# segasai/rvspecfit

Hardware: AMD Instinct MI355X
Metric: spectra/sec (CCF+chi2 grid) DESI 3-arm (higher is better)
Workload: dtype f64

## Files before the change

### include/rvsgpu.h

```cpp
#ifndef RVSGPU_H
#define RVSGPU_H
#include <stdint.h>

#ifdef __cplusplus
extern "C" {
#endif

#define RVS_E_ARG (-1)
#define RVS_E_LAUNCH (-2)

#define RVS_ST_SPLINE_RANGE 0x1
#define RVS_ST_SPLINE_GRID 0x2
#define RVS_ST_NONFINITE 0x4
#define RVS_ST_CHOL_FALLBACK 0x8
#define RVS_ST_OUTSIDE_NAN 0x10
#define RVS_ST_CCF_FAILED 0x20
#define RVS_ST_ALLMASKED 0x40
#define RVS_ST_QUAD_ASSERT 0x80
#define RVS_ST_ILLCOND 0x100
#define RVS_ST_NONPOS_MEDIAN 0x200
#define RVS_ST_RBF_NOTPD 0x400

#define RVS_ABI_VERSION 18
int rvs_abi_version(void);
// ... 303 lines not shown
int rvs_grid_moments(const double *chisq, const double *vels,
                     int64_t vel_stride, const int32_t *nvel, int G, int Np,
                     int Nv, int quadratic, double *res, double *probs,
                     int32_t *status, void *stream);

int rvs_ccf_preprocess(const double *lam, const double *spec,
                       const double *espec, const uint8_t *badmask, int npix,
                       int B, int continuum, const double *Eb, const int32_t *El,
                       const double *Cinv, const int32_t *istart, int nnode,
                       const int32_t *bin_start, const int32_t *xind,
                       const double *rw, int nfft, double maxerr,
                       double *proc_spec, double *proc_ivar, double *sse,
                       double *cont, double *pfit, int32_t *status,
                       void *stream);
int rvs_ccf_preprocess_g(const double *lam, const double *spec, const double *espec,
                         const uint8_t *badmask, int npix, int B, int continuum,
                         const double *Eb, const int32_t *El, const double *Cinv,
                         const int32_t *istart, int nnode,
                         const int32_t *bin_start, const int32_t *xind,
                         const double *rw, int nfft, double maxerr,
                         double *proc_spec, double *proc_ivar, double *sse,
                         double *cont, double *pfit, int32_t *status,
                         const int32_t *grid_id, const int32_t *npix_g,
                         const int32_t *nnode_g, void *stream);

int rvs_ccf_fft_pos(int nfft, int f);
int rvs_ccf_xcorr(const double *proc_spec, const double *proc_ivar, int nfft,
                  int B, const double *tfft, const double *tfft2, int T,
                  const double *twid, int continuum, const int32_t *lag_pos,
                  const double *lag_vel, int nlag, const int32_t *ilo,
                  const double *vgrid, int nvel, double beta,
                  const uint8_t *prune, double *chisq, double *work,
                  void *stream);

#define RVS_CCF_MODEL_MAX_NTP 9216
int rvs_ccf_model_rows(const float *dats, int64_t ngrid, const int64_t *sel,
                       int exp_flag, int ntp, int M, double *rows, void *stream);
int rvs_ccf_models_build(const double *rows, const uint8_t *f32row,
                         const double *erows, int ntp, int M, int continuum,
                         const double *Eb, const int32_t *El, const double *Cinv,
                         const int32_t *istart, int nnode, const int32_t *bin_start,
                         const double *lnlam, const double *logl, const int32_t *ihi,
                         int npoints, const double *twid, double *model, double *fft,
                         double *fft2, double *cont, double *pfit, int32_t *status,
                         void *stream);

int rvs_ccf_select(const double *chisq, const double *sse, int narm_sse, int B,
                   int T, const double *vgrid, int nvel, double *res,
                   double *best_ccf, int32_t *status, void *stream);

int rvs_template_nn(const double *params, int B, int ndim, uint32_t log_mask,
                    const double *M, const double *S, int nlayer,
                    const float *const *W, const float *const *b,
                    const int32_t *dims, float *act0, float *act1,
                    double *templ, void *stream);

int rvs_template_nn_grad(const double *params, int B, int ndim, uint32_t log_mask,
                         const double *M, const double *S, int nlayer,
                         const float *const *W, const float *const *b,
                         const int32_t *dims, float *act0, float *act1,
                         double *templ , void *stream);

int rvs_nn_outside(const double *params, int B, int ndim, uint32_t log_mask,
                   const double *M, const double *S, int mapped,
                   const double *xeqs, int nfx, const double *yeqs, int nfy,
                   double *outside, void *stream);
// ... 294 lines not shown
```

### rvspecfit_amd/_lib.py

```python
import ctypes
import os

import torch

_HERE = os.path.dirname(os.path.abspath(__file__))
LIB_PATH = os.path.join(_HERE, 'librvsgpu.so')

P = ctypes.c_void_p
I = ctypes.c_int
L = ctypes.c_int64
D = ctypes.c_double
U = ctypes.c_uint32

SIGNATURES = {
    'rvs_abi_version': (I, []),
    'rvs_option_set': (I, [ctypes.c_char_p, I]),
    'rvs_option_get': (I, [ctypes.c_char_p, P]),
    'rvs_template_polylinear': (I, [P, L, I, P, P, P, I, P, P, U, I, P, I, P, P,
                                    P, P, P]),
    'rvs_template_polylinear_grad': (I, [P, L, I, P, P, P, I, P, P, U, I, P, I, P,
                                         P, P, P, P]),
    'rvs_template_tri': (I, [P, I, P, P, P, I, I, U, I, P, I, P, P, P, P, P]),
    'rvs_template_tri_buckets': (I, [P, I, P, P, P, I, I, U, I, P, P, I, P, P, P,
                                     P, P]),
# ... 76 lines not shown
    'rvs_lm_run': (I, [P, P, P, P, I, P, P]),
    'rvs_epoch_map': (I, [I, I, I, I, P, P, P, P, P, I, P, P, P, P, P, D, D, D, P, P, P,
                          P, P, P, P, P]),
    'rvs_epoch_finish': (I, [I, I, I, I, P, I, P, P, P, P, P, P, P, P, P, P, P, P, I, P,
                             P, D, P, P, P]),
    'rvs_alm_row_size': (L, [I, I]),
    'rvs_alm_begin': (P, [I, I, P, P, D, D, D, D, I]),
    'rvs_alm_pending': (L, [P, P, P, L]),
    'rvs_alm_feed': (I, [P, P, L]),
    'rvs_alm_result': (I, [P, P, P, P, P, P, P, P, P, P]),
    'rvs_alm_end': (None, [P]),
    'rvs_alm_run_bytes': (L, []),
    'rvs_alm_run': (I, [P, P, P, P]),
    'rvs_objective_max_ntp': (I, [I]),
    'rvs_objective_resol_ok': (I, [I, I, I, I]),
    'rvs_objective_work_size': (L, [I, I]),
    'rvs_objective_fused': (I, [P, I, I, P, P, P, I, P, D, I, P, P, P, P]),
    'rvs_objective_from_template': (I, [P, I, I, P, P, P, P, I, P, D, I, P, P, P,
                                        P]),
    'rvs_objective_fused_n': (I, [P, I, I, P, P, P, I, P, P, D, I, P, P, P, P]),
    'rvs_objective_from_template_n': (I, [P, I, I, P, P, P, P, I, P, P, D, I, P,
                                          P, P, P]),
    'rvs_grid_moments': (I, [P, P, L, P, I, I, I, I, P, P, P, P]),
    'rvs_basis_build': (I, [P, P, I, I, I, I, P, P, P, P, P]),
    'rvs_ccf_tables_build': (I, [P, P, I, I, P, I, I, P, P, P, I, P, P, P, P, P, P,
                                 P]),
    'rvs_ccf_preprocess': (I, [P, P, P, P, I, I, I, P, P, P, P, I, P, P, P, I, D,
                               P, P, P, P, P, P, P]),
    'rvs_ccf_preprocess_g': (I, [P, P, P, P, I, I, I, P, P, P, P, I, P, P, P, I,
                                 D, P, P, P, P, P, P, P, P, P, P]),
    'rvs_ccf_fft_pos': (I, [I, I]),
    'rvs_ccf_xcorr': (I, [P, P, I, I, P, P, I, P, I, P, P, I, P, P, I, D, P, P,
                          P, P]),
    'rvs_ccf_select': (I, [P, P, I, I, I, P, I, P, P, P, P]),
    'rvs_ccf_model_rows': (I, [P, L, P, I, I, I, P, P]),
    'rvs_ccf_models_build': (I, [P, P, P, I, I, I, P, P, P, P, I, P, P, P, P, I, P,
                                 P, P, P, P, P, P, P]),
    'rvs_template_nn': (I, [P, I, I, U, P, P, I, P, P, P, P, P, P, P]),
    'rvs_template_nn_grad': (I, [P, I, I, U, P, P, I, P, P, P, P, P, P, P]),
    'rvs_template_nn_arms': (I, [P, I, I, I, P, P]),
    'rvs_template_nn_arms_n': (I, [P, I, P, I, I, P, P]),
    'rvs_nn_outside': (I, [P, I, I, U, P, P, I, P, I, P, I, P, P]),
    'rvs_rebin_weights': (I, [P, I, P, P, P, P, I, I, P, P]),
    'rvs_rebin_apply': (I, [P, I, L, I, I, P, P, I, P, P, P, I, I, P, P]),
    'rvs_template_normalize': (I, [P, I, I, P, I, D, D, I, I, P, P, P, P]),
    'rvs_rbf_work_size': (L, [I, I]),
    'rvs_rbf_factor': (I, [P, I, I, D, P, P, P, P]),
    'rvs_rbf_solve': (I, [P, I, L, I, I, P, P, P]),
    'rvs_rbf_eval': (I, [P, I, P, I, I, D, P, I, I, P, L, P]),
    'rvs_nn_train_work_size': (L, [I, I, I, P]),
    'rvs_nn_train_grad': (I, [P, P, I, P, I, I, P, P, P, P, P, D, P, P, P, P, P, P]),
    'rvs_nn_adam_step': (I, [I, P, P, P, P, P, P, P, P, P, D, I, P]),
    'rvs_nn_train_epoch': (I, [P, P, I, P, I, I, I, P, P, P, P, P, P, P, P, P, D, D, I,
                               P, P, P, P]),
}

_lib = None
ABI_VERSION = 18


class RvsGpuError(RuntimeError):
    pass


def lib():
    global _lib
# ... 207 lines not shown
```

### rvspecfit_amd/csrc/ccf_fft.hip

```cpp
#include "common.h"

#define XC_NT 512
#define XC_NTW(n2) ((n2) >> 3)

struct XcLds {
  int t1;
  int c0;
  int t1c;
  int ca;
  int lt;
  size_t bytes;
};
#define XW_NT1C 73
#define XW_NLT 256
#define XC_LDS_MAX (159 * 1024)
__host__ __device__ constexpr XcLds xc_lds_pair(int n2, int nlag) {
  const int t1 = n2, c0 = t1 + XC_NTW(n2);
  return {t1, c0, 0, 0, 0,
          sizeof(double2) * (size_t)c0 + sizeof(double) * 2 * (size_t)nlag};
}
__host__ __device__ constexpr XcLds xc_lds_ws(int n2, int nlag, bool ratio) {
  const int t1 = 2 * n2, c0 = t1 + XC_NTW(n2), t1c = c0 + ((nlag + 1) >> 1),
            ca = t1c + XW_NT1C, lt = ca + (ratio ? (nlag + 1) >> 1 : 0);
  return {t1, c0, t1c, ca, lt,
          sizeof(double2) * (size_t)lt + sizeof(int32_t) * (size_t)XW_NLT};
}
__host__ __device__ constexpr XcLds xc_lds_ws2(int n2, int nlag) {
  const int t1 = 4 * n2, c0 = t1 + XC_NTW(n2);
  return {t1, c0, 0, 0, 0,
          sizeof(double2) * (size_t)c0 + sizeof(double) * 2 * (size_t)nlag};
}
__host__ __device__ constexpr bool xc_lds_fits(const XcLds &L, int n2, int nimg,
                                               int nrow, int nlag, bool ws, bool ratio) {
  const size_t D2 = sizeof(double2), D = sizeof(double);
  size_t end = D2 * (size_t)nimg * n2;
  if (D2 * L.t1 < end) return false;
  end = D2 * (L.t1 + XC_NTW(n2));
  if (D2 * L.c0 < end) return false;
  end = D2 * L.c0 + D * (size_t)nrow * nlag;
  if (ws) {
    if (D2 * L.t1c < end) return false;
    end = D2 * (L.t1c + 72);
    if (D2 * L.ca < end) return false;
    end = D2 * L.ca + (ratio ? D * (size_t)nlag : 0);
    if (D2 * L.lt < end) return false;
    end = D2 * L.lt + sizeof(int32_t) * (size_t)XW_NLT;
  }
  return end <= L.bytes && L.bytes <= XC_LDS_MAX;
}
constexpr bool xc_lds_check() {
  for (int nlag = 2; nlag <= 512; nlag++)
    for (int n2 = 2048; n2 <= 4096; n2 *= 2) {
      for (int ratio = 0; ratio < 2; ratio++)
        if (!xc_lds_fits(xc_lds_ws(n2, nlag, ratio), n2, 2, 1, nlag, true, ratio))
          return false;
      if (n2 == 2048 && !xc_lds_fits(xc_lds_ws2(n2, nlag), n2, 4, 2, nlag, false, false))
        return false;
      if (!xc_lds_fits(xc_lds_pair(n2, nlag), n2, 1, 2, nlag, false, false))
        return false;
    }
  return true;
}
static_assert(xc_lds_check(), "an LDS array of a cross-correlation kernel overlaps "
                              "its neighbour or ends beyond the launch's request");

__device__ __forceinline__ double2 cmul(double2 a, double2 b) {
  return make_double2(a.x * b.x - a.y * b.y, a.x * b.y + a.y * b.x);
}
__device__ __forceinline__ double2 cadd(double2 a, double2 b) {
  return make_double2(a.x + b.x, a.y + b.y);
}
__device__ __forceinline__ double2 csub(double2 a, double2 b) {
  return make_double2(a.x - b.x, a.y - b.y);
}
template <int SIGN>
__device__ __forceinline__ double2 cmuli(double2 a) {
  return (SIGN > 0) ? make_double2(-a.y, a.x) : make_double2(a.y, -a.x);
}

__host__ __device__ inline int xc_plan(int log2n, int *rad) {
  int n = 0, l = log2n;
  while (l >= 3) {
    rad[n++] = 8;
    l -= 3;
  }
  if (l == 2) rad[n++] = 4;
  if (l == 1) rad[n++] = 2;
  return n;
// ... 519 lines not shown
    if (pre) {
      if (tid < nlag) dst[tid] = fr[pre_pos] * inv_n;
    } else {
      for (int l = tid; l < nlag; l += XB_NT) dst[l] = fr[lag_pos[l]] * inv_n;
    }
    __syncthreads();
  }
  if (!continuum) {
    for (int l = tid; l < nlag; l += XB_NT) c0[l] = -c0[l] * c0[l] / c1[l];
    __syncthreads();
  }
  if (pre) {
    if (tid < nvel) {
      const double sl = (c0[pre_lo + 1] - c0[pre_lo]) / (pre_x1 - pre_x0);
      const double val = sl * (pre_xg - pre_x0) + c0[pre_lo];
      out[tid] = (beta != 0.0) ? beta * pre_old + val : val;
    }
    XC_T(2);
    return;
  }
  for (int v = tid; v < nvel; v += XB_NT) {
    const int lo = ilo[v];
    const double x0 = lag_vel[lo], x1 = lag_vel[lo + 1];
    const double sl = (c0[lo + 1] - c0[lo]) / (x1 - x0);
    const double val = sl * (vgrid[v] - x0) + c0[lo];
    out[v] = (beta != 0.0) ? beta * out[v] + val : val;
  }
}


#define XW_NT 1024
#define XW_HALF 512

template <int SIGN, int LOG2N>
__device__ __forceinline__ void xw_pass(double2 *a, const double2 *T1, int p, int t,
                                        const double2 *Tc = nullptr) {
  const int lgM = LOG2N - 3 * p, lgMp = lgM - 3, Mp = 1 << lgMp;
  const int tws = LOG2N + 1 - lgM;
  const int blk = t >> lgMp, r = t & (Mp - 1);
  const int base = (blk << lgM) + r;
  double2 v[8];
#pragma unroll
  for (int j = 0; j < 8; j++) v[j] = a[base + Mp * j];
  dft8<SIGN>(v);
  if (Mp > 1) {
    double2 w1 = Tc ? Tc[r] : T1[r << (tws - 1)];
    if (SIGN < 0) w1.y = -w1.y;
    v[1] = cmul(v[1], w1);
    const double2 w2 = cmul(w1, w1);
    v[2] = cmul(v[2], w2);
    double2 wc = cmul(w2, w1);
    v[3] = cmul(v[3], wc);
    const double2 w4 = cmul(w2, w2);
    v[4] = cmul(v[4], w4);
    v[7] = cmul(v[7], cmul(w4, wc));
    wc = cmul(w4, w1);
    v[5] = cmul(v[5], wc);
    v[6] = cmul(v[6], cmul(w4, w2));
  }
#pragma unroll
  for (int q = 0; q < 8; q++) a[base + Mp * q] = v[q];
}

template <int LOG2N, bool RATIO>
__global__ void __launch_bounds__(XW_NT)
    ccf_xcorr_ws_kernel(const double2 *__restrict__ work,
                        const double2 *__restrict__ tfft,
                        const double2 *__restrict__ tfft2, int T,
                        const double2 *__restrict__ tw,
                        const int32_t *__restrict__ lag_pos,
                        const double *__restrict__ lag_vel, int nlag,
                        const int32_t *__restrict__ ilo,
                        const double *__restrict__ vgrid, int nvel, double beta,
                        const uint8_t *__restrict__ prune,
                        double *__restrict__ chisq) {
  extern __shared__ double2 fa[];
  constexpr int log2n = LOG2N, n2 = 1 << LOG2N, nfft = 2 * n2, npair = n2 / 2;
  constexpr int NPP = npair / XW_HALF;
  constexpr bool P12 = (LOG2N == 12);
  static_assert(LOG2N == 12 || LOG2N == 11, "plans 8,8,8,8 and 8,8,8,4 only");
  auto img = [&](int i) -> double2 * { return fa + (i & 1) * n2; };
  const XcLds lds = xc_lds_ws(n2, nlag, RATIO);
  const double2 *T1 = fa + lds.t1;
  double *c0 = reinterpret_cast<double *>(fa + lds.c0);
  double2 *T1c = fa + lds.t1c;
  double *cA = reinterpret_cast<double *>(fa + lds.ca);
  int32_t *lt = reinterpret_cast<int32_t *>(fa + lds.lt);
  const int TI = RATIO ? 2 * T : T;
  const int b = blockIdx.x, tid = threadIdx.x;
  const bool producer = tid >= XW_HALF;
  const int pt = tid & (XW_HALF - 1);
  const double inv_n = 1.0 / nfft;
  if (P12 && tid < 72)
    T1c[tid] = tid < 64 ? tw[2 * (tid << 3)] : tw[2 * ((tid - 64) << (log2n - 6))];
  xc_fill_twiddles<XW_NT>(fa + n2, n2, tw);
  XcMasks pmask = {0u, 0u, 0u};
  bool bad = !P12;
  if (P12 && !producer) {
    pmask = xc_load_masks<XW_HALF>(prune, n2);
    const int pos8 = pt & 7;
    const unsigned m = pmask.g;
    bad = m != 0 && !((pos8 == 0 && m == 0x01u) || (pos8 == 7 && m == 0x80u));
  }
  if (P12 && tid < XW_NLT) lt[tid] = -1;
  const bool fold = !__syncthreads_or(bad);
  if (P12) {
    if (fold && tid < nlag) {
      const int p = lag_pos[tid], e = (p >> 1) & 63;
      if (e == 0 || e == 63) lt[(((p >> 7) & 63) << 2) + (e ? 2 : 0) + (p & 1)] = tid;
    }
    __syncthreads();
  }
  const double2 *Sc = work + ((int64_t)b * 2) * (n2 + 1);
  const double2 *Vc = Sc + (n2 + 1);
  typedef int v4i_t __attribute__((ext_vector_type(4)));
  auto ld = [](const __amdgpu_buffer_rsrc_t &r, int off) {
    const v4i_t v = __builtin_amdgcn_raw_buffer_load_b128(r, off, 0, 0);
    return make_double2(__hiloint2double(v.y, v.x), __hiloint2double(v.w, v.z));
  };
  const int nbytes = (n2 + 1) * 16;
  if (producer) {
    double2 Sk[NPP], Vk[NPP], Sm[NPP], Vm[NPP];
#pragma unroll
    for (int u = 0; u < NPP; u++) {
      const int k = 1 + pt + u * XW_HALF, m = n2 - k;
      Sk[u] = Sc[k], Vk[u] = Vc[k], Sm[u] = Sc[m], Vm[u] = Vc[m];
    }
// ... 27 lines not shown
      const int k = 1 + ptv + u * XW_HALF, m = n2 - k;
      double2 Xk, Xm;
      if (RATIO) {
        const bool second = (tcur & 1) != 0;
        Xk = cmul(o[0], second ? Vk[u] : Sk[u]);
        Xm = cmul(o[2], second ? Vm[u] : Sm[u]);
      } else {
        const double2 p1 = cmul(o[0], Sk[u]), p2 = cmul(o[1], Vk[u]);
        Xk = make_double2(p2.x - 2 * p1.x, p2.y - 2 * p1.y);
        const double2 q1 = cmul(o[2], Sm[u]), q2 = cmul(o[3], Vm[u]);
        Xm = make_double2(q2.x - 2 * q1.x, q2.y - 2 * q1.y);
      }
      const double2 e = make_double2(Xk.x + Xm.x, Xk.y - Xm.y);
      const double2 d = make_double2(Xk.x - Xm.x, Xk.y + Xm.y);
      const double2 q = cmul(o[4], d);
      dst[k] = make_double2(e.x - q.y, e.y + q.x);
      if (m != k) dst[m] = make_double2(e.x + q.y, -e.y + q.x);
      if (u == NPP - 1 && ptv == 0) {
        double xk, xm;
        if (RATIO) {
          const bool second = (tcur & 1) != 0;
          xk = cmul(second ? dc[1] : dc[0], second ? Vc[0] : Sc[0]).x;
          xm = cmul(second ? dc[3] : dc[2], second ? Vc[n2] : Sc[n2]).x;
        } else {
          const double2 a1 = cmul(dc[0], Sc[0]), a2 = cmul(dc[1], Vc[0]);
          const double2 b1 = cmul(dc[2], Sc[n2]), b2 = cmul(dc[3], Vc[n2]);
          xk = a2.x - 2 * a1.x, xm = b2.x - 2 * b1.x;
        }
        dst[0] = make_double2(xk + xm, xk - xm);
      }
    };
    const bool two = P12 && fold;
    const int nbar = two ? 2 : 5;
    issue(0, 0, op[0]);
    if (NPP == 2) issue(0, 1, op[1]);
    for (int it = -1; it < TI; it++) {
      const int tn = it + 1;
      if (tn < TI) {
        double2 *dst = img(tn);
        {
          const int tt = RATIO ? (tn >> 1) : tn;
          const double2 *Fp = tfft + (int64_t)tt * (n2 + 1);
          const double2 *F2p = tfft2 + (int64_t)tt * (n2 + 1);
          dc[0] = Fp[0], dc[1] = F2p[0], dc[2] = Fp[n2], dc[3] = F2p[n2];
        }
        if (NPP == 2) {
#pragma unroll
          for (int u = 0; u < 2; u++) {
            form(dst, u, op[u], tn);
            if (tn + 1 < TI) issue(tn + 1, u, op[u]);
            __syncthreads();
          }
        } else {
#pragma unroll
          for (int u = 0; u < NPP; u++) {
            if (u + 1 < NPP)
              issue(tn, u + 1, op[(u + 1) & 1]);
            else if (tn + 1 < TI)
              issue(tn + 1, 0, op[(u + 1) & 1]);
            form(dst, u, op[u & 1], tn);
            if (!two || (u & 1)) __syncthreads();
          }
        }
        for (int q = two ? NPP / 2 : NPP; q < nbar; q++) __syncthreads();
      } else {
        for (int q = 0; q < nbar; q++) __syncthreads();
      }
    }
    return;
  }
  const int tvx = min(pt, nvel - 1);
  const int pre_pos = lag_pos[min(pt, nlag - 1)];
  const int pre_lo = ilo[tvx];
  const double pre_xg = vgrid[tvx];
  const double pre_x0 = lag_vel[pre_lo], pre_x1 = lag_vel[pre_lo + 1];
  typedef int v4i32_t __attribute__((ext_vector_type(4)));
  v4i32_t lag = {-1, -1, -1, -1};
  if (P12) lag = reinterpret_cast<const v4i32_t *>(lt)[pt >> 3];
  for (int it = -1; it < TI; it++) {
    if (it < 0) {
      const int nbar = (P12 && fold) ? 2 : 5;
      for (int q = 0; q < nbar; q++) __syncthreads();
      continue;
    }
    double2 *a = img(it);
    double *out = chisq + ((int64_t)b * T + (RATIO ? (it >> 1) : it)) * nvel;
    double pre_old = 0;
    if (beta != 0.0) pre_old = out[tvx];
    if (pt < (n2 >> 3)) xw_pass<1, LOG2N>(a, T1, 0, pt);
    __syncthreads();
    if (pt < (n2 >> 3)) xw_pass<1, LOG2N>(a, T1, 1, pt, P12 ? T1c : nullptr);
    if (P12 && fold) {
      __builtin_amdgcn_fence(__ATOMIC_RELEASE, "wavefront");
      __builtin_amdgcn_wave_barrier();
      __builtin_amdgcn_fence(__ATOMIC_ACQUIRE, "wavefront");
      const int s = pt & 7;
      const int B = pt >> 3;
      const unsigned m0 = pmask.b0 & 1u, m63 = pmask.b7 >> 7;
      if (m0 | m63) {
        double2 v[8];
#pragma unroll
        for (int j = 0; j < 8; j++) v[j] = a[B * 64 + s + 8 * j];
        dft8<1>(v);
        double2 w = T1c[64 + s];
        w.y = -w.y;
        double2 x63 = cmul(v[7], w), x0 = v[0];
        auto sum8 = [](double x) {
          x += dpp_get<0xb1, 0xf, 0xf>(x);
          x += dpp_get<0x4e, 0xf, 0xf>(x);
          x += dpp_get<0x141, 0xf, 0xf>(x);
          return x;
        };
        auto put = [&](int l, double x) {
          if (l < 0) return;
          const double c = x * inv_n;
          if (!RATIO)
            c0[l] = c;
          else if (it & 1)
            c0[l] = -cA[l] * cA[l] / c;
          else
            cA[l] = c;
        };
        if (m0) {
          x0.x = sum8(x0.x);
// ... 200 lines not shown
    xw_pass<1, LOG2N>(a, T1, 0, bt);
    __syncthreads();
    xw_pass<1, LOG2N>(a, T1, 1, bt);
    __syncthreads();
    xw_pass<1, LOG2N>(a, T1, 2, bt);
    __syncthreads();
#pragma unroll
    for (int h = 0; h < 2; h++) {
      const int base = (bt + 256 * h) << 2;
      double2 v0 = a[base], v1 = a[base + 1], v2 = a[base + 2], v3 = a[base + 3];
      dft4<1>(v0, v1, v2, v3);
      a[base] = v0, a[base + 1] = v1, a[base + 2] = v2, a[base + 3] = v3;
    }
    __syncthreads();
    if (pt < nlag) {
      c0[pt] = reinterpret_cast<const double *>(img(it, 0))[pre_pos[0]] * inv_n;
      c0[nlag + pt] = reinterpret_cast<const double *>(img(it, 1))[pre_pos[0]] * inv_n;
    }
    __syncthreads();
    if (pt < nvel) {
      const double dx = pre_x1 - pre_x0, xg = pre_xg - pre_x0;
      const double sl0 = (c0[pre_lo + 1] - c0[pre_lo]) / dx;
      const double val0 = sl0 * xg + c0[pre_lo];
      out0[pt] = (beta != 0.0) ? beta * old0 + val0 : val0;
      if (two) {
        const double sl1 = (c0[nlag + pre_lo + 1] - c0[nlag + pre_lo]) / dx;
        const double val1 = sl1 * xg + c0[nlag + pre_lo];
        out1[pt] = (beta != 0.0) ? beta * old1 + val1 : val1;
      }
    }
  }
}

extern "C" int rvs_ccf_xcorr(const double *proc_spec, const double *proc_ivar,
                             int nfft, int B, const double *tfft,
                             const double *tfft2, int T, const double *twid_,
                             int continuum, const int32_t *lag_pos,
                             const double *lag_vel, int nlag, const int32_t *ilo,
                             const double *vgrid, int nvel, double beta,
                             const uint8_t *prune, double *chisq, double *work,
                             void *stream) {
  int log2n = 0;
  while ((2 << log2n) < nfft) log2n++;
  if ((2 << log2n) != nfft || nfft < 64 || nfft > 16384) return RVS_E_ARG;
  if (B < 1 || T < 1 || T > 65535 || nlag < 2 || nvel < 1) return RVS_E_ARG;
  const int n2 = nfft >> 1;
  const size_t shm1 = xc_lds_pair(n2, 0).bytes;
  const size_t shm2 = xc_lds_pair(n2, nlag).bytes;
  if (shm2 > XC_LDS_MAX) return RVS_E_ARG;
  hipStream_t st = rvs_stream(stream);
  const double2 *tw = reinterpret_cast<const double2 *>(twid_);
  static bool attr_set = false;
  if (!attr_set) {
    (void)hipFuncSetAttribute((const void *)ccf_rfft_kernel<false>,
                              hipFuncAttributeMaxDynamicSharedMemorySize,
                              XC_LDS_MAX);
    (void)hipFuncSetAttribute((const void *)ccf_xcorr_kernel,
                              hipFuncAttributeMaxDynamicSharedMemorySize,
                              XC_LDS_MAX);
    (void)hipGetLastError();
    attr_set = true;
  }
  hipLaunchKernelGGL(ccf_rfft_kernel<false>, dim3(B, 2), dim3(XC_NT), shm1, st,
                     proc_spec, proc_ivar, nfft, log2n, tw,
                     reinterpret_cast<double2 *>(work), (double2 *)nullptr);
  RVS_LAUNCH_CHECK();
  const int G = xc_group(T, nfft);
  {
    const bool ws_on = rvs_opt(RVS_OPT_XC_WS) != 0;
    const bool p12 = (nfft == 8192 && prune), p11 = (nfft == 4096);
    if (ws_on && (p12 || p11) && nlag <= XW_HALF && nvel <= XW_HALF && T >= 2) {
      static bool ws_attr = false;
      if (!ws_attr) {
        (void)hipFuncSetAttribute((const void *)ccf_xcorr_ws_kernel<12, false>,
                                  hipFuncAttributeMaxDynamicSharedMemorySize,
                                  XC_LDS_MAX);
        (void)hipFuncSetAttribute((const void *)ccf_xcorr_ws_kernel<12, true>,
                                  hipFuncAttributeMaxDynamicSharedMemorySize,
                                  XC_LDS_MAX);
        (void)hipFuncSetAttribute((const void *)ccf_xcorr_ws_kernel<11, true>,
                                  hipFuncAttributeMaxDynamicSharedMemorySize,
                                  XC_LDS_MAX);
        (void)hipFuncSetAttribute((const void *)ccf_xcorr_ws2_kernel,
                                  hipFuncAttributeMaxDynamicSharedMemorySize,
                                  XC_LDS_MAX);
        (void)hipGetLastError();
        ws_attr = true;
      }
      const size_t shmw = xc_lds_ws(n2, nlag, !continuum).bytes;
#define RVS_XW_ARGS                                                                 \
  reinterpret_cast<const double2 *>(work), reinterpret_cast<const double2 *>(tfft),  \
      reinterpret_cast<const double2 *>(tfft2), T, tw, lag_pos, lag_vel, nlag, ilo,  \
      vgrid, nvel, beta, prune, chisq
      if (!continuum) {
        if (p12)
          hipLaunchKernelGGL((ccf_xcorr_ws_kernel<12, true>), dim3(B), dim3(XW_NT), shmw,
                             st, RVS_XW_ARGS);
        else
          hipLaunchKernelGGL((ccf_xcorr_ws_kernel<11, true>), dim3(B), dim3(XW_NT), shmw,
                             st, RVS_XW_ARGS);
        RVS_LAUNCH_CHECK();
        return 0;
      }
      if (p12)
        hipLaunchKernelGGL((ccf_xcorr_ws_kernel<12, false>), dim3(B), dim3(XW_NT), shmw, st,
                           reinterpret_cast<const double2 *>(work),
                           reinterpret_cast<const double2 *>(tfft),
                           reinterpret_cast<const double2 *>(tfft2), T, tw, lag_pos,
                           lag_vel, nlag, ilo, vgrid, nvel, beta, prune, chisq);
      else
        hipLaunchKernelGGL(ccf_xcorr_ws2_kernel, dim3(B), dim3(XW_NT),
                           xc_lds_ws2(n2, nlag).bytes, st,
                           reinterpret_cast<const double2 *>(work),
                           reinterpret_cast<const double2 *>(tfft),
                           reinterpret_cast<const double2 *>(tfft2), T, tw, lag_pos,
                           lag_vel, nlag, ilo, vgrid, nvel, beta, chisq);
      RVS_LAUNCH_CHECK();
      return 0;
    }
  }
  const int bmax = G ? (int)(0x7fffffffll / xc_nblocks(T, 1, G)) : 65535;
  for (int b0 = 0; b0 < B; b0 += bmax) {
    const int nb = (B - b0 < bmax) ? (B - b0) : bmax;
    const dim3 grid = G ? dim3((unsigned)xc_nblocks(T, nb, G)) : dim3(T, nb);
    hipLaunchKernelGGL(
        ccf_xcorr_kernel, grid, dim3(XB_NT), shm2, st,
        reinterpret_cast<const double2 *>(work) + (int64_t)b0 * 2 * (n2 + 1),
        nfft, log2n, reinterpret_cast<const double2 *>(tfft),
        reinterpret_cast<const double2 *>(tfft2), T, tw, continuum, lag_pos,
        lag_vel, nlag, ilo, vgrid, nvel, beta, prune,
        chisq + (int64_t)b0 * T * nvel, nb, G);
    RVS_LAUNCH_CHECK();
  }
  return 0;
}
```

### rvspecfit_amd/csrc/options.cpp

```cpp
#include <atomic>
#include <cstdlib>
#include <cstring>
#include <mutex>

#include "options.h"

namespace {
struct OptDef {
  const char *name;
  const char *env;
  int dflt;
};
const OptDef kDefs[RVS_OPT_COUNT] = {
    {"xc_ws", "RVS_XC_WS", 1},
    {"obj_inblk_max", "RVS_OBJ_INBLK_MAX", 768},
    {"obj_sort", "RVS_OBJ_SORT", 1},
    {"nn_pipe", "RVS_NN_PIPE", 1},
    {"nm_split_min", "RVS_NM_SPLIT_MIN", 1024},
    {"nm_spec_max", "RVS_NM_SPEC_MAX", 21},
    {"nm_tail_window", "RVS_NM_TAIL_WINDOW", 16},
    {"cg_tab", "RVS_CG_TAB", 1},
};
std::atomic<int> g_val[RVS_OPT_COUNT];
std::once_flag g_once;

void init_table() {
  for (int i = 0; i < RVS_OPT_COUNT; i++) {
    int v = kDefs[i].dflt;
    if (const char *ev = std::getenv(kDefs[i].env))
      v = std::atoi(ev);
    g_val[i].store(v, std::memory_order_relaxed);
  }
}
int find(const char *name) {
  if (!name) return -1;
  for (int i = 0; i < RVS_OPT_COUNT; i++)
    if (!std::strcmp(name, kDefs[i].name)) return i;
  return -1;
}
}

int rvs_opt(int id) {
  std::call_once(g_once, init_table);
  return g_val[id].load(std::memory_order_relaxed);
}

extern "C" int rvs_option_set(const char *name, int value) {
  const int i = find(name);
  if (i < 0) return RVS_E_ARG;
  std::call_once(g_once, init_table);
  g_val[i].store(value, std::memory_order_relaxed);
  return 0;
}

// ... 7 lines not shown
```

### rvspecfit_amd/csrc/options.h

```cpp
#pragma once
#include "../../include/rvsgpu.h"

enum {
  RVS_OPT_XC_WS,
  RVS_OPT_OBJ_INBLK_MAX,
  RVS_OPT_OBJ_SORT,
  RVS_OPT_NN_PIPE,
  RVS_OPT_NM_SPLIT_MIN,
  RVS_OPT_NM_SPEC_MAX,
  RVS_OPT_NM_TAIL_WINDOW,
  RVS_OPT_CG_TAB,
  RVS_OPT_COUNT
};
int rvs_opt(int id);
```

### rvspecfit_amd/engine.py

```python
import ctypes
import threading

import numpy as np
import torch

from . import _lib
from . import ccf_tables

SPEED_OF_LIGHT = 299792.458

KTIMERS = None


class _ktime:

    def __init__(self, name, units=1):
        self.name, self.units = name, units

    def __enter__(self):
        if KTIMERS is not None:
            self.e0 = torch.cuda.Event(enable_timing=True)
            self.e0.record()

    def __exit__(self, *a):
# ... 1243 lines not shown
        _lib.ptr(status), arm.grid_args()[0], _lib.ptr(T['npix_g']),
        _lib.ptr(T['nnode_g']), _lib.stream())
    _lib.check(rc, 'rvs_ccf_preprocess')
    out = dict(proc_spec=ps, proc_ivar=pi, sse=sse, status=status)
    if details:
        out.update(cont=cont, pfit=pfit)
    return out


def ccf_fit(batch, libs, config, keep_all=False, max_chunk=None):
    L = _lib.lib()
    dev = batch.device
    S = batch.S
    ref = libs[batch.names[0]].ccf_set(config)
    Tn = ref['T']
    for n in batch.names[1:]:
        cc = libs[n].ccf_set(config)
        if cc['T'] != Tn:
            raise RuntimeError('CCF template counts are inconsistent across setups')
        if (not np.array_equal(ref['params'], cc['params'])
                or not np.array_equal(ref['vsinis'], cc['vsinis'],
                                      equal_nan=True)):
            raise RuntimeError('The parameters of the CCF templates do not match')
    tabs = [a.ccf_tables(libs[a.name], config) for a in batch.arms]
    nvel = len(tabs[0]['vgrid_host'])
    pre = [ccf_preprocess(a, libs[a.name], config) for a in batch.arms]
    sse = torch.stack([p['sse'] for p in pre]).contiguous()
    status = torch.zeros(S, dtype=torch.int32, device=dev)
    for p in pre:
        status |= p['status']
    if max_chunk is None:
        max_chunk = max(1, min(S, int(2e9 // (Tn * nvel * 8))))
        nchunk = -(-S // max_chunk)
        max_chunk = -(-S // nchunk)
    res = torch.empty((S, 4), dtype=torch.float64, device=dev)
    best_ccf = torch.empty((S, nvel), dtype=torch.float64, device=dev)
    allchi = None
    for a, b in _chunks(S, max_chunk):
        n = b - a
        acc = torch.empty((n, Tn, nvel), dtype=torch.float64, device=dev)
        for ia, arm in enumerate(batch.arms):
            cc = libs[arm.name].ccf_set(config)
            T = tabs[ia]
            nfft = cc['npoints']
            work = torch.empty((n, 2, nfft // 2 + 1, 2), dtype=torch.float64,
                               device=dev)
            with _ktime('ccf_xcorr', n):
              rc = L.rvs_ccf_xcorr(
                _lib.ptr(pre[ia]['proc_spec'][a:b]),
                _lib.ptr(pre[ia]['proc_ivar'][a:b]), nfft, n,
                _lib.ptr(cc['fft']), _lib.ptr(cc['fft2']), Tn,
                _lib.ptr(T['twid']), int(cc['continuum']),
                _lib.ptr(T['lag_pos']), _lib.ptr(T['lag_vel']), T['nlag'],
                _lib.ptr(T['ilo']), _lib.ptr(T['vgrid']), nvel,
                0.0 if ia == 0 else 1.0, _lib.ptr(T['prune']), _lib.ptr(acc),
                _lib.ptr(work), _lib.stream())
            _lib.check(rc, 'rvs_ccf_xcorr')
        sse_c = sse[:, a:b].contiguous()
        rc = L.rvs_ccf_select(_lib.ptr(acc), _lib.ptr(sse_c), len(batch.arms),
                              n, Tn, _lib.ptr(tabs[0]['vgrid']), nvel,
                              _lib.ptr(res[a:b]), _lib.ptr(best_ccf[a:b]),
                              _lib.ptr(status[a:b]), _lib.stream())
        _lib.check(rc, 'rvs_ccf_select')
        if keep_all:
            allchi = acc + sse_c.sum(dim=0)[:, None, None]
    out = dict(best_id=res[:, 0].long(), best_vel=res[:, 1].contiguous(),
               best_pix=res[:, 2].long(), best_ccf=best_ccf, status=status,
# ... 8 lines not shown
```

Measured before the change: 84490.

## Split tail batch blocks across templates and precompute twiddle powers in LDS

```diff
diff --git a/include/rvsgpu.h b/include/rvsgpu.h
--- a/include/rvsgpu.h
+++ b/include/rvsgpu.h
@@ -359,6 +359,8 @@
                   const double *vgrid, int nvel, double beta,
                   const uint8_t *prune, double *chisq, double *work,
                   void *stream);
+int rvs_ccf_xcorr_plan(int nfft, int B, int T, int nlag, int continuum, int ncu,
+                       int32_t *out);
 
 #define RVS_CCF_MODEL_MAX_NTP 9216
 int rvs_ccf_model_rows(const float *dats, int64_t ngrid, const int64_t *sel,
diff --git a/rvspecfit_amd/_lib.py b/rvspecfit_amd/_lib.py
--- a/rvspecfit_amd/_lib.py
+++ b/rvspecfit_amd/_lib.py
@@ -132,6 +132,7 @@
     'rvs_ccf_fft_pos': (I, [I, I]),
     'rvs_ccf_xcorr': (I, [P, P, I, I, P, P, I, P, I, P, P, I, P, P, I, D, P, P,
                           P, P]),
+    'rvs_ccf_xcorr_plan': (I, [I, I, I, I, I, I, P]),
     'rvs_ccf_select': (I, [P, P, I, I, I, P, I, P, P, P, P]),
     'rvs_ccf_model_rows': (I, [P, L, P, I, I, I, P, P]),
     'rvs_ccf_models_build': (I, [P, P, P, I, I, I, P, P, P, P, I, P, P, P, P, I, P,
diff --git a/rvspecfit_amd/csrc/ccf_fft.hip b/rvspecfit_amd/csrc/ccf_fft.hip
--- a/rvspecfit_amd/csrc/ccf_fft.hip
+++ b/rvspecfit_amd/csrc/ccf_fft.hip
@@ -5,6 +5,7 @@
 
 struct XcLds {
   int t1;
+  int p1;
   int c0;
   int t1c;
   int ca;
@@ -16,18 +17,21 @@
 #define XC_LDS_MAX (159 * 1024)
 __host__ __device__ constexpr XcLds xc_lds_pair(int n2, int nlag) {
   const int t1 = n2, c0 = t1 + XC_NTW(n2);
-  return {t1, c0, 0, 0, 0,
+  return {t1, 0, c0, 0, 0, 0,
           sizeof(double2) * (size_t)c0 + sizeof(double) * 2 * (size_t)nlag};
 }
-__host__ __device__ constexpr XcLds xc_lds_ws(int n2, int nlag, bool ratio) {
+#define XW_NP1 384
+__host__ __device__ constexpr XcLds xc_lds_ws(int n2, int nlag, bool ratio,
+                                              bool p1 = false) {
   const int t1 = 2 * n2, c0 = t1 + XC_NTW(n2), t1c = c0 + ((nlag + 1) >> 1),
-            ca = t1c + XW_NT1C, lt = ca + (ratio ? (nlag + 1) >> 1 : 0);
-  return {t1, c0, t1c, ca, lt,
-          sizeof(double2) * (size_t)lt + sizeof(int32_t) * (size_t)XW_NLT};
+            ca = t1c + XW_NT1C, lt = ca + (ratio ? (nlag + 1) >> 1 : 0),
+            pp = lt + (int)(sizeof(int32_t) * XW_NLT / sizeof(double2));
+  return {t1, p1 ? pp : 0, c0, t1c, ca, lt,
+          sizeof(double2) * (size_t)(pp + (p1 ? XW_NP1 : 0))};
 }
 __host__ __device__ constexpr XcLds xc_lds_ws2(int n2, int nlag) {
   const int t1 = 4 * n2, c0 = t1 + XC_NTW(n2);
-  return {t1, c0, 0, 0, 0,
+  return {t1, 0, c0, 0, 0, 0,
           sizeof(double2) * (size_t)c0 + sizeof(double) * 2 * (size_t)nlag};
 }
 __host__ __device__ constexpr bool xc_lds_fits(const XcLds &L, int n2, int nimg,
@@ -45,6 +49,10 @@
     end = D2 * L.ca + (ratio ? D * (size_t)nlag : 0);
     if (D2 * L.lt < end) return false;
     end = D2 * L.lt + sizeof(int32_t) * (size_t)XW_NLT;
+    if (L.p1) {
+      if (D2 * L.p1 < end) return false;
+      end = D2 * (L.p1 + XW_NP1);
+    }
   }
   return end <= L.bytes && L.bytes <= XC_LDS_MAX;
 }
@@ -52,8 +60,10 @@
   for (int nlag = 2; nlag <= 512; nlag++)
     for (int n2 = 2048; n2 <= 4096; n2 *= 2) {
       for (int ratio = 0; ratio < 2; ratio++)
-        if (!xc_lds_fits(xc_lds_ws(n2, nlag, ratio), n2, 2, 1, nlag, true, ratio))
-          return false;
+        for (int p1 = 0; p1 < (n2 == 4096 ? 2 : 1); p1++) {
+          const XcLds L = xc_lds_ws(n2, nlag, ratio, p1);
+          if (!xc_lds_fits(L, n2, 2, 1, nlag, true, ratio)) return false;
+        }
       if (n2 == 2048 && !xc_lds_fits(xc_lds_ws2(n2, nlag), n2, 4, 2, nlag, false, false))
         return false;
       if (!xc_lds_fits(xc_lds_pair(n2, nlag), n2, 1, 2, nlag, false, false))
@@ -639,9 +649,30 @@
 #define XW_NT 1024
 #define XW_HALF 512
 
+struct XwPowers {
+  double2 w2, w3, w4, w5, w6, w7;
+};
+__device__ __forceinline__ XwPowers xw_powers(double2 w1) {
+  XwPowers w;
+  w.w2 = cmul(w1, w1);
+  w.w3 = cmul(w.w2, w1);
+  w.w4 = cmul(w.w2, w.w2);
+  w.w7 = cmul(w.w4, w.w3);
+  w.w5 = cmul(w.w4, w1);
+  w.w6 = cmul(w.w4, w.w2);
+  return w;
+}
+template <bool W1>
+__device__ __forceinline__ double2 cmul_as_chain(double2 v, double2 w) {
+#pragma clang fp contract(off)
+  const double re = v.y * w.y, im = W1 ? v.x * w.y : v.y * w.x;
+  return make_double2(__builtin_fma(v.x, w.x, -re),
+                      W1 ? __builtin_fma(v.y, w.x, im) : __builtin_fma(v.x, w.y, im));
+}
 template <int SIGN, int LOG2N>
 __device__ __forceinline__ void xw_pass(double2 *a, const double2 *T1, int p, int t,
-                                        const double2 *Tc = nullptr) {
+                                        const double2 *Tc = nullptr,
+                                        const double2 *Pw = nullptr) {
   const int lgM = LOG2N - 3 * p, lgMp = lgM - 3, Mp = 1 << lgMp;
   const int tws = LOG2N + 1 - lgM;
   const int blk = t >> lgMp, r = t & (Mp - 1);
@@ -650,7 +681,11 @@
 #pragma unroll
   for (int j = 0; j < 8; j++) v[j] = a[base + Mp * j];
   dft8<SIGN>(v);
-  if (Mp > 1) {
+  if (Mp > 1 && Pw) {
+    v[1] = cmul_as_chain<true>(v[1], Tc[r]);
+#pragma unroll
+    for (int q = 2; q < 8; q++) v[q] = cmul_as_chain<false>(v[q], Pw[(q - 2) * Mp + r]);
+  } else if (Mp > 1) {
     double2 w1 = Tc ? Tc[r] : T1[r << (tws - 1)];
     if (SIGN < 0) w1.y = -w1.y;
     v[1] = cmul(v[1], w1);
@@ -669,7 +704,7 @@
   for (int q = 0; q < 8; q++) a[base + Mp * q] = v[q];
 }
 
-template <int LOG2N, bool RATIO>
+template <int LOG2N, bool RATIO, bool P1 = false>
 __global__ void __launch_bounds__(XW_NT)
     ccf_xcorr_ws_kernel(const double2 *__restrict__ work,
                         const double2 *__restrict__ tfft,
@@ -680,26 +715,41 @@
                         const int32_t *__restrict__ ilo,
                         const double *__restrict__ vgrid, int nvel, double beta,
                         const uint8_t *__restrict__ prune,
-                        double *__restrict__ chisq) {
+                        double *__restrict__ chisq, int nfull, int parts) {
   extern __shared__ double2 fa[];
   constexpr int log2n = LOG2N, n2 = 1 << LOG2N, nfft = 2 * n2, npair = n2 / 2;
   constexpr int NPP = npair / XW_HALF;
   constexpr bool P12 = (LOG2N == 12);
   static_assert(LOG2N == 12 || LOG2N == 11, "plans 8,8,8,8 and 8,8,8,4 only");
+  static_assert(P12 || !P1, "the LDS table belongs to the plan 8,8,8,8");
   auto img = [&](int i) -> double2 * { return fa + (i & 1) * n2; };
-  const XcLds lds = xc_lds_ws(n2, nlag, RATIO);
+  const XcLds lds = xc_lds_ws(n2, nlag, RATIO, P1);
   const double2 *T1 = fa + lds.t1;
   double *c0 = reinterpret_cast<double *>(fa + lds.c0);
   double2 *T1c = fa + lds.t1c;
   double *cA = reinterpret_cast<double *>(fa + lds.ca);
   int32_t *lt = reinterpret_cast<int32_t *>(fa + lds.lt);
-  const int TI = RATIO ? 2 * T : T;
-  const int b = blockIdx.x, tid = threadIdx.x;
+  double2 *Pw = P1 ? fa + lds.p1 : nullptr;
+  const int tid = threadIdx.x;
+  int b = blockIdx.x, i0 = 0, i1 = T;
+  if (b >= nfull) {
+    const int j = b - nfull, part = j % parts;
+    b = nfull + j / parts;
+    i0 = (int)((int64_t)part * T / parts), i1 = (int)((int64_t)(part + 1) * T / parts);
+  }
+  if (RATIO) i0 *= 2, i1 *= 2;
   const bool producer = tid >= XW_HALF;
   const int pt = tid & (XW_HALF - 1);
   const double inv_n = 1.0 / nfft;
-  if (P12 && tid < 72)
-    T1c[tid] = tid < 64 ? tw[2 * (tid << 3)] : tw[2 * ((tid - 64) << (log2n - 6))];
+  if (P12 && tid < 72) {
+    const double2 w1 = tid < 64 ? tw[2 * (tid << 3)] : tw[2 * ((tid - 64) << (log2n - 6))];
+    T1c[tid] = w1;
+    if (P1 && tid < 64) {
+      const XwPowers w = xw_powers(w1);
+      Pw[tid] = w.w2, Pw[64 + tid] = w.w3, Pw[128 + tid] = w.w4;
+      Pw[192 + tid] = w.w5, Pw[256 + tid] = w.w6, Pw[320 + tid] = w.w7;
+    }
+  }
   xc_fill_twiddles<XW_NT>(fa + n2, n2, tw);
   XcMasks pmask = {0u, 0u, 0u};
   bool bad = !P12;
@@ -793,11 +843,11 @@
     };
     const bool two = P12 && fold;
     const int nbar = two ? 2 : 5;
-    issue(0, 0, op[0]);
-    if (NPP == 2) issue(0, 1, op[1]);
-    for (int it = -1; it < TI; it++) {
+    issue(i0, 0, op[0]);
+    if (NPP == 2) issue(i0, 1, op[1]);
+    for (int it = i0 - 1; it < i1; it++) {
       const int tn = it + 1;
-      if (tn < TI) {
+      if (tn < i1) {
         double2 *dst = img(tn);
         {
           const int tt = RATIO ? (tn >> 1) : tn;
@@ -809,7 +859,7 @@
 #pragma unroll
           for (int u = 0; u < 2; u++) {
             form(dst, u, op[u], tn);
-            if (tn + 1 < TI) issue(tn + 1, u, op[u]);
+            if (tn + 1 < i1) issue(tn + 1, u, op[u]);
             __syncthreads();
           }
         } else {
@@ -817,7 +867,7 @@
           for (int u = 0; u < NPP; u++) {
             if (u + 1 < NPP)
               issue(tn, u + 1, op[(u + 1) & 1]);
-            else if (tn + 1 < TI)
+            else if (tn + 1 < i1)
               issue(tn + 1, 0, op[(u + 1) & 1]);
             form(dst, u, op[u & 1], tn);
             if (!two || (u & 1)) __syncthreads();
@@ -838,8 +888,8 @@
   typedef int v4i32_t __attribute__((ext_vector_type(4)));
   v4i32_t lag = {-1, -1, -1, -1};
   if (P12) lag = reinterpret_cast<const v4i32_t *>(lt)[pt >> 3];
-  for (int it = -1; it < TI; it++) {
-    if (it < 0) {
+  for (int it = i0 - 1; it < i1; it++) {
+    if (it < i0) {
       const int nbar = (P12 && fold) ? 2 : 5;
       for (int q = 0; q < nbar; q++) __syncthreads();
       continue;
@@ -850,7 +900,7 @@
     if (beta != 0.0) pre_old = out[tvx];
     if (pt < (n2 >> 3)) xw_pass<1, LOG2N>(a, T1, 0, pt);
     __syncthreads();
-    if (pt < (n2 >> 3)) xw_pass<1, LOG2N>(a, T1, 1, pt, P12 ? T1c : nullptr);
+    if (pt < (n2 >> 3)) xw_pass<1, LOG2N>(a, T1, 1, pt, P12 ? T1c : nullptr, Pw);
     if (P12 && fold) {
       __builtin_amdgcn_fence(__ATOMIC_RELEASE, "wavefront");
       __builtin_amdgcn_wave_barrier();
@@ -1117,6 +1167,63 @@
   }
 }
 
+enum { XC_FORM_PAIR, XC_FORM_WS12, XC_FORM_WS12R, XC_FORM_WS2, XC_FORM_WS11R };
+enum { XC_PLAN_FORM, XC_PLAN_ZERO, XC_PLAN_P1, XC_PLAN_LDS, XC_PLAN_FULL, XC_PLAN_REM,
+       XC_PLAN_PARTS, XC_PLAN_BLOCKS };
+static int xc_launch_plan(int nfft, int B, int T, int nlag, int nvel, int continuum,
+                          bool pruned, int ncu, int32_t out[8]) {
+  int log2n = 0;
+  while ((2 << log2n) < nfft) log2n++;
+  if ((2 << log2n) != nfft || nfft < 64 || nfft > 16384) return RVS_E_ARG;
+  if (B < 1 || T < 1 || T > 65535 || nlag < 2 || nvel < 1 || !out) return RVS_E_ARG;
+  const int n2 = nfft >> 1;
+  if (xc_lds_pair(n2, nlag).bytes > XC_LDS_MAX) return RVS_E_ARG;
+  const bool p12 = (nfft == 8192 && pruned), p11 = (nfft == 4096);
+  const bool ws = rvs_opt(RVS_OPT_XC_WS) != 0 && (p12 || p11) && nlag <= XW_HALF &&
+                  nvel <= XW_HALF && T >= 2;
+  const int64_t nblk = ws ? B : (int64_t)B * T;
+  out[XC_PLAN_FORM] = !ws ? XC_FORM_PAIR
+                      : p12 ? (continuum ? XC_FORM_WS12 : XC_FORM_WS12R)
+                            : (continuum ? XC_FORM_WS2 : XC_FORM_WS11R);
+  out[XC_PLAN_ZERO] = out[XC_PLAN_P1] = out[XC_PLAN_REM] = 0;
+  out[XC_PLAN_FULL] = ws ? B : 0;
+  out[XC_PLAN_PARTS] = 1;
+  out[XC_PLAN_BLOCKS] = (int32_t)(nblk < 0x7fffffff ? nblk : 0x7fffffff);
+  if (!ws) {
+    out[XC_PLAN_LDS] = (int32_t)xc_lds_pair(n2, nlag).bytes;
+  } else if (!p12) {
+    out[XC_PLAN_LDS] = (int32_t)(continuum ? xc_lds_ws2(n2, nlag).bytes
+                                           : xc_lds_ws(n2, nlag, true).bytes);
+  } else {
+    const XcLds L = xc_lds_ws(n2, nlag, !continuum, rvs_opt(RVS_OPT_XC_P1_LDS) != 0);
+    out[XC_PLAN_P1] = L.p1 != 0;
+    out[XC_PLAN_LDS] = (int32_t)L.bytes;
+    const int rem = ncu > 0 ? B % ncu : 0;
+    const int parts = rem ? (T < ncu / rem ? T : ncu / rem) : 1;
+    if (parts >= 2) {
+      out[XC_PLAN_FULL] = B - rem;
+      out[XC_PLAN_REM] = rem;
+      out[XC_PLAN_PARTS] = parts;
+      out[XC_PLAN_BLOCKS] = B - rem + rem * parts;
+    }
+  }
+  return 0;
+}
+
+extern "C" int rvs_ccf_xcorr_plan(int nfft, int B, int T, int nlag, int continuum,
+                                  int ncu, int32_t *out) {
+  return xc_launch_plan(nfft, B, T, nlag, 1, continuum, true, ncu, out);
+}
+
+typedef void (*XwKernel)(const double2 *, const double2 *, const double2 *, int,
+                         const double2 *, const int32_t *, const double *, int,
+                         const int32_t *, const double *, int, double, const uint8_t *,
+                         double *, int, int);
+static const XwKernel kXwKernels[5] = {
+    ccf_xcorr_ws_kernel<12, false, false>, ccf_xcorr_ws_kernel<12, false, true>,
+    ccf_xcorr_ws_kernel<12, true, false>, ccf_xcorr_ws_kernel<12, true, true>,
+    ccf_xcorr_ws_kernel<11, true>};
+
 extern "C" int rvs_ccf_xcorr(const double *proc_spec, const double *proc_ivar,
                              int nfft, int B, const double *tfft,
                              const double *tfft2, int T, const double *twid_,
@@ -1125,14 +1232,25 @@
                              const double *vgrid, int nvel, double beta,
                              const uint8_t *prune, double *chisq, double *work,
                              void *stream) {
+  int ncu = rvs_opt(RVS_OPT_XC_SPLIT_CUS);
+  int32_t plan[8];
+  int rc = xc_launch_plan(nfft, B, T, nlag, nvel, continuum, prune != nullptr, ncu, plan);
+  if (rc) return rc;
+  if (ncu == 0 &&
+      (plan[XC_PLAN_FORM] == XC_FORM_WS12 || plan[XC_PLAN_FORM] == XC_FORM_WS12R)) {
+    int dev = 0;
+    if (hipGetDevice(&dev) == hipSuccess &&
+        hipDeviceGetAttribute(&ncu, hipDeviceAttributeMultiprocessorCount, dev) ==
+            hipSuccess)
+      rc = xc_launch_plan(nfft, B, T, nlag, nvel, continuum, true, ncu, plan);
+    (void)hipGetLastError();
+  }
+  if (rc) return rc;
   int log2n = 0;
   while ((2 << log2n) < nfft) log2n++;
-  if ((2 << log2n) != nfft || nfft < 64 || nfft > 16384) return RVS_E_ARG;
-  if (B < 1 || T < 1 || T > 65535 || nlag < 2 || nvel < 1) return RVS_E_ARG;
   const int n2 = nfft >> 1;
   const size_t shm1 = xc_lds_pair(n2, 0).bytes;
   const size_t shm2 = xc_lds_pair(n2, nlag).bytes;
-  if (shm2 > XC_LDS_MAX) return RVS_E_ARG;
   hipStream_t st = rvs_stream(stream);
   const double2 *tw = reinterpret_cast<const double2 *>(twid_);
   static bool attr_set = false;
@@ -1151,58 +1269,40 @@
                      reinterpret_cast<double2 *>(work), (double2 *)nullptr);
   RVS_LAUNCH_CHECK();
   const int G = xc_group(T, nfft);
-  {
-    const bool ws_on = rvs_opt(RVS_OPT_XC_WS) != 0;
-    const bool p12 = (nfft == 8192 && prune), p11 = (nfft == 4096);
-    if (ws_on && (p12 || p11) && nlag <= XW_HALF && nvel <= XW_HALF && T >= 2) {
-      static bool ws_attr = false;
-      if (!ws_attr) {
-        (void)hipFuncSetAttribute((const void *)ccf_xcorr_ws_kernel<12, false>,
-                                  hipFuncAttributeMaxDynamicSharedMemorySize,
-                                  XC_LDS_MAX);
-        (void)hipFuncSetAttribute((const void *)ccf_xcorr_ws_kernel<12, true>,
-                                  hipFuncAttributeMaxDynamicSharedMemorySize,
-                                  XC_LDS_MAX);
-        (void)hipFuncSetAttribute((const void *)ccf_xcorr_ws_kernel<11, true>,
-                                  hipFuncAttributeMaxDynamicSharedMemorySize,
-                                  XC_LDS_MAX);
-        (void)hipFuncSetAttribute((const void *)ccf_xcorr_ws2_kernel,
-                                  hipFuncAttributeMaxDynamicSharedMemorySize,
-                                  XC_LDS_MAX);
-        (void)hipGetLastError();
-        ws_attr = true;
-      }
-      const size_t shmw = xc_lds_ws(n2, nlag, !continuum).bytes;
-#define RVS_XW_ARGS                                                                 \
-  reinterpret_cast<const double2 *>(work), reinterpret_cast<const double2 *>(tfft),  \
-      reinterpret_cast<const double2 *>(tfft2), T, tw, lag_pos, lag_vel, nlag, ilo,  \
-      vgrid, nvel, beta, prune, chisq
-      if (!continuum) {
-        if (p12)
-          hipLaunchKernelGGL((ccf_xcorr_ws_kernel<12, true>), dim3(B), dim3(XW_NT), shmw,
-                             st, RVS_XW_ARGS);
-        else
-          hipLaunchKernelGGL((ccf_xcorr_ws_kernel<11, true>), dim3(B), dim3(XW_NT), shmw,
-                             st, RVS_XW_ARGS);
-        RVS_LAUNCH_CHECK();
-        return 0;
-      }
-      if (p12)
-        hipLaunchKernelGGL((ccf_xcorr_ws_kernel<12, false>), dim3(B), dim3(XW_NT), shmw, st,
-                           reinterpret_cast<const double2 *>(work),
-                           reinterpret_cast<const double2 *>(tfft),
-                           reinterpret_cast<const double2 *>(tfft2), T, tw, lag_pos,
-                           lag_vel, nlag, ilo, vgrid, nvel, beta, prune, chisq);
-      else
-        hipLaunchKernelGGL(ccf_xcorr_ws2_kernel, dim3(B), dim3(XW_NT),
-                           xc_lds_ws2(n2, nlag).bytes, st,
-                           reinterpret_cast<const double2 *>(work),
-                           reinterpret_cast<const double2 *>(tfft),
-                           reinterpret_cast<const double2 *>(tfft2), T, tw, lag_pos,
-                           lag_vel, nlag, ilo, vgrid, nvel, beta, chisq);
-      RVS_LAUNCH_CHECK();
-      return 0;
-    }
+  const int form = plan[XC_PLAN_FORM];
+  if (form != XC_FORM_PAIR) {
+    static bool ws_attr = false;
+    if (!ws_attr) {
+      for (const XwKernel k : kXwKernels)
+        (void)hipFuncSetAttribute((const void *)k,
+                                  hipFuncAttributeMaxDynamicSharedMemorySize, XC_LDS_MAX);
+      (void)hipFuncSetAttribute((const void *)ccf_xcorr_ws2_kernel,
+                                hipFuncAttributeMaxDynamicSharedMemorySize, XC_LDS_MAX);
+      (void)hipGetLastError();
+      ws_attr = true;
+    }
+    const dim3 grid(plan[XC_PLAN_BLOCKS]);
+    const size_t shmw = plan[XC_PLAN_LDS];
+    if (form == XC_FORM_WS2) {
+      hipLaunchKernelGGL(ccf_xcorr_ws2_kernel, grid, dim3(XW_NT), shmw, st,
+                         reinterpret_cast<const double2 *>(work),
+                         reinterpret_cast<const double2 *>(tfft),
+                         reinterpret_cast<const double2 *>(tfft2), T, tw, lag_pos,
+                         lag_vel, nlag, ilo, vgrid, nvel, beta, chisq);
+    } else {
+      const XwKernel k =
+          form == XC_FORM_WS11R
+              ? kXwKernels[4]
+              : kXwKernels[2 * (form == XC_FORM_WS12R) + plan[XC_PLAN_P1]];
+      hipLaunchKernelGGL(k, grid, dim3(XW_NT), shmw, st,
+                         reinterpret_cast<const double2 *>(work),
+                         reinterpret_cast<const double2 *>(tfft),
+                         reinterpret_cast<const double2 *>(tfft2), T, tw, lag_pos,
+                         lag_vel, nlag, ilo, vgrid, nvel, beta, prune, chisq,
+                         plan[XC_PLAN_FULL], plan[XC_PLAN_PARTS]);
+    }
+    RVS_LAUNCH_CHECK();
+    return 0;
   }
   const int bmax = G ? (int)(0x7fffffffll / xc_nblocks(T, 1, G)) : 65535;
   for (int b0 = 0; b0 < B; b0 += bmax) {
diff --git a/rvspecfit_amd/csrc/options.cpp b/rvspecfit_amd/csrc/options.cpp
--- a/rvspecfit_amd/csrc/options.cpp
+++ b/rvspecfit_amd/csrc/options.cpp
@@ -20,6 +20,8 @@
     {"nm_spec_max", "RVS_NM_SPEC_MAX", 21},
     {"nm_tail_window", "RVS_NM_TAIL_WINDOW", 16},
     {"cg_tab", "RVS_CG_TAB", 1},
+    {"xc_p1_lds", "RVS_XC_P1_LDS", 1},
+    {"xc_split_cus", "RVS_XC_SPLIT_CUS", 0},
 };
 std::atomic<int> g_val[RVS_OPT_COUNT];
 std::once_flag g_once;
diff --git a/rvspecfit_amd/csrc/options.h b/rvspecfit_amd/csrc/options.h
--- a/rvspecfit_amd/csrc/options.h
+++ b/rvspecfit_amd/csrc/options.h
@@ -10,6 +10,8 @@
   RVS_OPT_NM_SPEC_MAX,
   RVS_OPT_NM_TAIL_WINDOW,
   RVS_OPT_CG_TAB,
+  RVS_OPT_XC_P1_LDS,
+  RVS_OPT_XC_SPLIT_CUS,
   RVS_OPT_COUNT
 };
 int rvs_opt(int id);
diff --git a/rvspecfit_amd/engine.py b/rvspecfit_amd/engine.py
--- a/rvspecfit_amd/engine.py
+++ b/rvspecfit_amd/engine.py
@@ -1299,7 +1299,12 @@
     if max_chunk is None:
         max_chunk = max(1, min(S, int(2e9 // (Tn * nvel * 8))))
         nchunk = -(-S // max_chunk)
+        bound = max_chunk
         max_chunk = -(-S // nchunk)
+        ncu = torch.cuda.get_device_properties(dev).multi_processor_count
+        whole = -(-max_chunk // ncu) * ncu
+        if whole <= bound:
+            max_chunk = whole
     res = torch.empty((S, 4), dtype=torch.float64, device=dev)
     best_ccf = torch.empty((S, nvel), dtype=torch.float64, device=dev)
     allchi = None
```

Result: no change. 85270 (median of 6 runs) (+0.9%).
